# REGRAGUIahmed/DGViT-Depth-Goal-Guided-Vision-Transformer-

Measured on AMD Instinct MI355X. Metric: depth frames/sec through DGViT fwd+bwd, batch 512x84x84, higher is better.
Workload: dtype f32

## Files before the change

### dgvit-depth-goal-guided-vision-transformer-_amd/_lib.py

```python
import ctypes
import os
from ctypes import POINTER, Structure, c_char_p, c_float, c_int, c_longlong, c_ulonglong, c_void_p

_HERE = os.path.dirname(os.path.abspath(__file__))
LIB_PATH = os.path.join(_HERE, "libdgvit_hip.so")
DIAG_LIB_PATH = os.path.join(_HERE, "libdgvit_hip_diag.so")


class DgvitError(RuntimeError):
    pass


class dgvit_config(Structure):
    _fields_ = [("image_h", c_int), ("image_w", c_int), ("patch_h", c_int), ("patch_w", c_int), ("dim", c_int),
                ("depth", c_int), ("heads", c_int), ("dim_head", c_int), ("mlp_dim", c_int), ("pool_mean", c_int), ("flags", c_int)]


FLAG_DENSE_LAST_BLOCK = 1
FLAG_WGRAD_OVERLAP = 2
FLAG_LONG_SEQUENCE = 4
MAPS_GOAL = 0
MAPS_ALL = 1


# ... 124 lines not shown
    "dgvit_got_bf16_backward_scratch_bytes": (_LL, [_CFG, _I]),
    "dgvit_got_backward_bf16": (_I, [_CFG, _TABLE, _P, _TABLE, _P, _P, _P, _P, _LL, _P, _LL, _I, _F, _ULL, _P, _P]),
    "dgvit_got_backward_bf16_ev": (_I, [_CFG, _TABLE, _P, _TABLE, _P, _P, _P, _P, _LL, _P, _LL, _I, _F, _ULL, _P, _P, POINTER(dgvit_grad_events)]),
    "dgvit_got_backward_bf16_v2": (_I, [_CFG, _TABLE, _P, _TABLE, _P, _P, _P, _P, _P, _LL, _P, _LL, _I, _F, _ULL, _P, _P]),
    "dgvit_got_backward_bf16_v2_ev": (_I, [_CFG, _TABLE, _P, _TABLE, _P, _P, _P, _P, _P, _LL, _P, _LL, _I, _F, _ULL, _P, _P,
                                           POINTER(dgvit_grad_events)]),
    "dgvit_wgrad_bf16_scratch_floats": (_LL, [_I, _I, _I]),
    "dgvit_wgrad_bf16": (_I, [_P, _P, _P, _P, _P, _LL, _I, _I, _I, _P]),
    "dgvit_cast_f32_bf16": (_I, [_P, _P, _LL, _P]),
    "dgvit_gemm_bf16": (_I, [_I, _P, _I, _P, _I, _P, _I, _I, _I, _I, _P, _P, _I, _P, _I, _P, _I, _P]),
    "dgvit_layernorm_forward_bf16": (_I, [_P, _P, _P, _P, _P, _P, _I, _I, _P]),
    "dgvit_attention_forward_bf16": (_I, [_P, _P, _P, _I, _I, _I, _I, _P]),
    "dgvit_got_forward_maps": (_I, [_CFG, _TABLE, _P, _P, _P, _P, _I, _P, _LL, _I, _F, _F, _ULL, _P, _P]),
    "dgvit_got_forward_maps_bf16": (_I, [_CFG, _TABLE, _P, _P, _P, _P, _P, _I, _P, _LL, _I, _F, _ULL, _P, _P]),
    "dgvit_attention_probs": (_I, [_P, _P, _P, _I, _I, _I, _I, _I, _P]),
    "dgvit_attention_probs_bf16": (_I, [_P, _P, _P, _I, _I, _I, _I, _I, _P]),
    "dgvit_attention_backward_bf16": (_I, [_P, _P, _P, _P, _P, _P, _I, _I, _I, _I, _P]),
    "dgvit_attention_forward_bf16_tiled": (_I, [_P, _P, _P, _I, _I, _I, _I, _I, _P]),
    "dgvit_attention_backward_bf16_tiled": (_I, [_P, _P, _P, _P, _P, _P, _I, _I, _I, _I, _P]),
    "dgvit_got_forward_bf16_v2": (_I, [_CFG, _TABLE, _P, _P, _P, _P, _P, _LL, _I, _I, _F, _F, _ULL, _P, _P]),
    "dgvit_got_forward_maps_bf16_v2": (_I, [_CFG, _TABLE, _P, _P, _P, _P, _P, _I, _P, _LL, _I, _F, _F, _ULL, _P, _P]),
    "dgvit_got_backward_bf16_v3": (_I, [_CFG, _TABLE, _P, _TABLE, _P, _P, _P, _P, _P, _LL, _P, _LL, _I, _F, _F, _ULL, _P, _P]),
    "dgvit_got_backward_bf16_v3_ev": (_I, [_CFG, _TABLE, _P, _TABLE, _P, _P, _P, _P, _P, _LL, _P, _LL, _I, _F, _F, _ULL, _P, _P,
                                           POINTER(dgvit_grad_events)]),
    "dgvit_attention_forward_bf16_tiled_drop": (_I, [_P, _P, _P, _I, _I, _I, _I, _I, _F, _ULL, _P, _I, _P]),
    "dgvit_attention_backward_bf16_tiled_drop": (_I, [_P, _P, _P, _P, _P, _P, _I, _I, _I, _I, _F, _ULL, _P, _I, _P]),
    "dgvit_drop_rows_bf16": (_I, [_P, _LL, _P, _LL, _LL, _I, _I, _F, _ULL, _P, _I, _I, _P]),
    "dgvit_profile_start": (_I, [_I]),
    "dgvit_profile_stop": (_I, [POINTER(ctypes.c_double), POINTER(ctypes.c_double), POINTER(c_longlong)]),
    "dgvit_profile_sampling": (_I, [_I]),
    "dgvit_profile_totals": (_I, [POINTER(ctypes.c_double), POINTER(c_longlong)]),
}
DIAG_SIGNATURES = {
    "dgvit_set_gemm_tile": (None, [_I]),
    "dgvit_set_grouped_reduce": (None, [_I]),
    "dgvit_set_gemm_split": (None, [_I]),
    "dgvit_set_gemm_lds_pad": (None, [_I]),
    "dgvit_set_ln_fusion": (None, [_I]),
    "dgvit_set_conv_gather": (None, [_I]),
    "dgvit_set_gemm_diagnostics": (None, [_I]),
    "dgvit_set_gemm_persistent": (None, [_I, _I]),
    "dgvit_gemm_persistent_launches": (ctypes.c_longlong, []),
    "dgvit_set_gemm_stamps": (None, [_P, _I]),
    "dgvit_set_small_batch_path": (None, [_I, _I]),
    "dgvit_set_block_path": (None, [_I, _I]),
    "dgvit_set_block_stamps": (None, [_P]),
    "dgvit_set_block_stamp_layer": (None, [_I]),
    "dgvit_set_gelu_grad_store": (None, [_I]),
    "dgvit_set_block_fuse": (None, [_I]),
    "dgvit_set_gemm_bf16_tile": (None, [_I]),
    "dgvit_set_gemm_bf16_group_m": (None, [_I]),
    "dgvit_set_gemm_bf16_l2_budget_kb": (None, [_I]),
    "dgvit_set_attention_bwd_single_pass": (None, [_I]),
    "dgvit_set_attention_single_query": (None, [_I]),
    "dgvit_set_last_block_fold": (None, [_I]),
    "dgvit_set_attention_bf16_long": (None, [_I]),
    "dgvit_set_attention_bf16_tiled_waves": (None, [_I]),
    "dgvit_set_gemm_wgrad_slice_major": (None, [_I]),
    "dgvit_attention_forward_queries": (_I, [_P, _P, _P, _I, _I, _I, _I, _I, _P]),
    "dgvit_attention_backward_queries": (_I, [_P, _P, _P, _P, _P, _I, _I, _I, _I, _I, _P]),
    "dgvit_attention_forward_bf16_queries": (_I, [_P, _P, _P, _I, _I, _I, _I, _I, _P]),
    "dgvit_set_gemm_bf16_mfma16": (None, [_I]),
    "dgvit_set_gemm_bf16_stamps": (None, [_P]),
    "dgvit_diag_layernorm_forward": (_I, [_P, _P, _P, _P, _P, _P, _I, _I, _I, _P]),
    "dgvit_diag_layernorm_backward": (_I, [_P, _P, _P, _P, _P, _P, _P, _P, _P, _P, _LL, _I, _I, _I, _I, _P]),
    "dgvit_diag_layernorm_forward_bf16": (_I, [_P, _P, _P, _P, _P, _P, _P, _P, _P, _I, _I, _I, _P]),
    "dgvit_diag_layernorm_backward_bf16": (_I, [_P, _P, _P, _P, _P, _P, _P, _P, _P, _P, _P, _LL, _I, _I, _I, _P]),
    "dgvit_diag_residual_add_bf16": (_I, [_P, _P, _P, _I, _I, _I, _P]),
    "dgvit_diag_transpose_cast_f32_bf16": (_I, [_P, _P, _I, _I, _P]),
    "dgvit_diag_colsum_scratch_floats": (_LL, [_I, _I]),
    "dgvit_diag_colsum": (_I, [_P, _LL, _P, _P, _LL, _I, _I, _I, _P]),
}
PROFILE_KINDS = 4

_lib = None
_product = None
_diag = None


def _open(path, signatures):
    if not os.path.exists(path):
        raise DgvitError(f"{path} not found: build it with `python {os.path.join(_HERE, 'build.py')}` "
                         "(hipcc --offload-arch=gfx950). There is no fallback path.")
    lib = ctypes.CDLL(path)
    for name, (res, args) in signatures.items():
        try:
            fn = getattr(lib, name)
        except AttributeError as e:
            raise DgvitError(f"{path} does not export {name}; rebuild it") from e
        fn.restype, fn.argtypes = res, args
    if lib.dgvit_abi_version() != ABI_VERSION:
        raise DgvitError(f"ABI mismatch: library {lib.dgvit_abi_version()} != binding {ABI_VERSION}")
    if lib.dgvit_config_size() != ctypes.sizeof(dgvit_config):
        raise DgvitError(f"dgvit_config is {ctypes.sizeof(dgvit_config)} bytes in the binding, {lib.dgvit_config_size()} in the library")
    return lib


def load():
    global _lib, _product
    if _lib is not None:
        return _lib
    if _product is None:
        _product = _open(LIB_PATH, SIGNATURES)
    _lib = _product
    return _lib

# ... 23 lines not shown
```

### dgvit-depth-goal-guided-vision-transformer-_amd/csrc/attention.hip

```cpp
#include "common.h"
#include "kernels.h"
#include "attention_tiles.h"

namespace {

template <int DH, int NW, int NKT_CT, bool DROP = false>
__global__ void __launch_bounds__(64 * NW, 2) attn_fwd_kernel(const float* __restrict__ qkv, float* __restrict__ out,
                                                              float* __restrict__ lse, int N, int H, float scale, int nq,
                                                              const LayerDrop drop) {
  constexpr int SK = DH + 4, DT = DH / 32, NTHR = 64 * NW;
  extern __shared__ __attribute__((aligned(16))) float smem[];
  const int nkt = NKT_CT ? NKT_CT : (N + 31) / 32, NP = nkt * 32;
  float* Ks = smem;
  float* Vs = smem + NP * SK;
  const int tid = threadIdx.x, lane = tid & 63, wave = tid >> 6;
  const int li = lane & 31, h = lane >> 5;
  const int b = blockIdx.x / H, hd = blockIdx.x % H;
  const int I = H * DH;
  const long long ld = 3ll * I;
  const float* base = qkv + (long long)b * N * ld + hd * DH;
  const float qscale = scale * DGVIT_LOG2E;

  const int nqt = (nq + 31) / 32;
  float4 qf[DH / 8];
// ... 346 lines not shown
  __syncthreads();
  for (int kt = wave; kt < nkt; kt += NW) {
    const int key = kt * 32 + li;
    const bool kv = key < N;
    if (kt != wave) {
      const int kc = kv ? key : 0;
      row_frags<DH>(kf, base + I + kc * ld, kv, h, 1.f);
      row_frags<DH>(vf, base + 2 * I + kc * ld, kv, h, 1.f);
    }
    f32x16 dk[DT], dv[DT];
    zero_tiles<DT>(dk);
    zero_tiles<DT>(dv);
#pragma unroll 1
    for (int qt = 0; qt < nqt; ++qt) {
      f32x16 s, dp;
#pragma unroll
      for (int r = 0; r < 16; ++r) {
        s[r] = 0.f;
        dp[r] = 0.f;
      }
      mfma_rows_x_frags<DH, SK>(s, X, qt * 32 + li, h, kf);
      mfma_rows_x_frags<DH, SK>(dp, Y, qt * 32 + li, h, vf);
#pragma unroll
      for (int r = 0; r < 16; ++r) {
        const int q = qt * 32 + acc_row(r, h);
        const float pv = (kv && q < nq) ? __builtin_amdgcn_exp2f(s[r] * qscale - lse_s[q]) : 0.f;
        float mk = 1.f;
        if constexpr (DROP) {
          if (kv && q < nq) {
            const uint4 rb = drop_bits((((long long)b * H + hd) * N + q) * ((N + 3) / 4) + key / 4, drop_seed(drop), drop.tag);
            const int w = key & 3;
            mk = drop_factor(w == 0 ? rb.x : w == 1 ? rb.y : w == 2 ? rb.z : rb.w, drop.keep, 1.0f / drop.keep);
          }
        }
        const float ds = DROP ? pv * (dp[r] * mk - del_s[q]) * scale : pv * (dp[r] - del_s[q]) * scale;
        const float pd = DROP ? pv * mk : pv;
        const float* dorow = Y + q * SK + li;
        const float* qrow = X + q * SK + li;
#pragma unroll
        for (int dt = 0; dt < DT; ++dt) {
          dv[dt] = __builtin_amdgcn_mfma_f32_32x32x2f32(dorow[dt * 32], pd, dv[dt], 0, 0, 0);
          dk[dt] = __builtin_amdgcn_mfma_f32_32x32x2f32(qrow[dt * 32], ds, dk[dt], 0, 0, 0);
        }
      }
    }
    if (kv) {
      store_T<DH>(dk, gbase + I + key * ld, h, 1.f);
      store_T<DH>(dv, gbase + 2 * I + key * ld, h, 1.f);
    }
  }
}

template <int DH>
__global__ void __launch_bounds__(256, 3) attn_bwd64_kernel(const float* __restrict__ qkv, const float* __restrict__ o_fwd,
                                                            const float* __restrict__ d_out, const float* __restrict__ lse,
                                                            float* __restrict__ dqkv, int N, int H, float scale) {
  constexpr int SK = DH + 4, DT = DH / 32, NP = 64, TQ = NP + 4;
  extern __shared__ __attribute__((aligned(16))) float smem[];
  float* X = smem;
  float* Y = X + NP * SK;
  float* T = Y + NP * SK;
  const int tid = threadIdx.x, lane = tid & 63, wave = tid >> 6;
  const int li = lane & 31, h = lane >> 5;
  const int b = blockIdx.x / H, hd = blockIdx.x % H;
  const int I = H * DH;
  const long long ld = 3ll * I;
  const float* base = qkv + (long long)b * N * ld + hd * DH;
  const float* obase = o_fwd + (long long)b * N * I + hd * DH;
  const float* dobase = d_out + (long long)b * N * I + hd * DH;
  float* gbase = dqkv + (long long)b * N * ld + hd * DH;
  const float qscale = scale * DGVIT_LOG2E;
  f32x16 dsT;
  const int qt1 = wave & 1, kt1 = wave >> 1, q1 = qt1 * 32 + li;
  {
    const int qt = qt1, kt = kt1, q = q1;
    const bool qv = q < N;
    const int qc = qv ? q : 0;
    float4 qf[DH / 8], dof[DH / 8];
    float delta, lq;
    {
      constexpr int C4 = DH / 4, PER = NP * C4 / 256;
      float4 kst[PER], vst[PER];
#pragma unroll
      for (int j = 0; j < PER; ++j) {
        const int f = tid + j * 256, row = f / C4, c = (f % C4) * 4;
        const int rr = row < N ? row : 0;
        kst[j] = *reinterpret_cast<const float4*>(base + I + rr * ld + c);
        vst[j] = *reinterpret_cast<const float4*>(base + 2 * I + rr * ld + c);
      }
      float4 of[DH / 8];
      row_frags<DH>(qf, base + qc * ld, qv, h, qscale);
      row_frags<DH>(dof, dobase + (long long)qc * I, qv, h, 1.f);
      row_frags<DH>(of, obase + (long long)qc * I, qv, h, 1.f);
      lq = qv ? lse[((long long)b * H + hd) * N + qc] : 0.f;
#pragma unroll
      for (int j = 0; j < PER; ++j) {
        const int f = tid + j * 256, row = f / C4, c = (f % C4) * 4;
        const float k = row < N ? 1.f : 0.f;
        *reinterpret_cast<float4*>(X + row * SK + c) = make_float4(kst[j].x * k, kst[j].y * k, kst[j].z * k, kst[j].w * k);
        *reinterpret_cast<float4*>(Y + row * SK + c) = make_float4(vst[j].x * k, vst[j].y * k, vst[j].z * k, vst[j].w * k);
      }
      float d = 0.f;
#pragma unroll
      for (int g = 0; g < DH / 8; ++g) d += (dof[g].x * of[g].x + dof[g].y * of[g].y) + (dof[g].z * of[g].z + dof[g].w * of[g].w);
      delta = d + __shfl_xor(d, 32, 64);
    }
    __syncthreads();
    f32x16 sT, dpT;
#pragma unroll
// ... 81 lines not shown
        for (int dt = 0; dt < DT; ++dt) dv[dt] = __builtin_amdgcn_mfma_f32_32x32x2f32(dov[e][dt], pe[e], dv[dt], 0, 0, 0);
    }
    __syncthreads();
#pragma unroll
    for (int r = 0; r < 16; ++r) T[(kt1 * 32 + acc_row(r, h)) * TQ + q1] = dsT[r];
    __syncthreads();
#pragma unroll
    for (int g = 0; g < 4; ++g) {
      if (qt * 32 + 8 * g >= N) continue;
      const float4 sf = *reinterpret_cast<const float4*>(T + key * TQ + qt * 32 + 8 * g + 4 * h);
      const float se[4] = {sf.x, sf.y, sf.z, sf.w};
      float qv4[4][DT];
#pragma unroll
      for (int e = 0; e < 4; ++e) {
        const float* qrow = X + (qt * 32 + 8 * g + 4 * h + e) * SK + li;
#pragma unroll
        for (int dt = 0; dt < DT; ++dt) qv4[e][dt] = qrow[dt * 32];
      }
#pragma unroll
      for (int e = 0; e < 4; ++e)
#pragma unroll
        for (int dt = 0; dt < DT; ++dt) dk[dt] = __builtin_amdgcn_mfma_f32_32x32x2f32(qv4[e][dt], se[e], dk[dt], 0, 0, 0);
    }
    __syncthreads();
    float* ek = T + key * TQ;
    float* ev = X + key * SK;
    if (qt == 1) {
#pragma unroll
      for (int dt = 0; dt < DT; ++dt)
#pragma unroll
        for (int c = 0; c < 4; ++c) {
          *reinterpret_cast<float4*>(ek + dt * 32 + 8 * c + 4 * h) = make_float4(dk[dt][4 * c], dk[dt][4 * c + 1], dk[dt][4 * c + 2], dk[dt][4 * c + 3]);
          *reinterpret_cast<float4*>(ev + dt * 32 + 8 * c + 4 * h) = make_float4(dv[dt][4 * c], dv[dt][4 * c + 1], dv[dt][4 * c + 2], dv[dt][4 * c + 3]);
        }
    }
    __syncthreads();
    if (qt == 0 && key < N) {
      const float unscale = 1.f / qscale;
#pragma unroll
      for (int dt = 0; dt < DT; ++dt)
#pragma unroll
        for (int c = 0; c < 4; ++c) {
          const float4 a = *reinterpret_cast<const float4*>(ek + dt * 32 + 8 * c + 4 * h);
          const float4 bq = *reinterpret_cast<const float4*>(ev + dt * 32 + 8 * c + 4 * h);
          *reinterpret_cast<float4*>(gbase + I + key * ld + dt * 32 + 8 * c + 4 * h) =
              make_float4((dk[dt][4 * c] + a.x) * unscale, (dk[dt][4 * c + 1] + a.y) * unscale, (dk[dt][4 * c + 2] + a.z) * unscale,
                          (dk[dt][4 * c + 3] + a.w) * unscale);
          *reinterpret_cast<float4*>(gbase + 2 * I + key * ld + dt * 32 + 8 * c + 4 * h) =
              make_float4(dv[dt][4 * c] + bq.x, dv[dt][4 * c + 1] + bq.y, dv[dt][4 * c + 2] + bq.z, dv[dt][4 * c + 3] + bq.w);
        }
    }
  }
}


template <int DH>
int launch_bwd64(const float* qkv, const float* o, const float* dout, const float* lse, float* dqkv, int B, int N, int H, float scale,
                 hipStream_t stream) {
  constexpr size_t lds = (size_t)(2 * 64 * (DH + 4) + 64 * 68) * sizeof(float);
  auto kern = attn_bwd64_kernel<DH>;
  TRY(allow_dynamic_lds<attn_bwd64_kernel<DH>>((int)lds, "attention_bwd"));
  {
    ProfileScope t(PROF_ATTN_BWD, 8.0 * B * H * (double)N * N * DH, stream);
    hipLaunchKernelGGL(kern, dim3(B * H), dim3(256), lds, stream, qkv, o, dout, lse, dqkv, N, H, scale);
  }
  DGVIT_CHECK_LAUNCH("attention_bwd64");
  return DGVIT_OK;
}

template <int W>
__device__ __forceinline__ float lanes_sum(float v) {
#pragma unroll
  for (int o = W >> 1; o > 0; o >>= 1) v += __shfl_xor(v, o, 64);
  return v;
}
template <int W>
__device__ __forceinline__ float groups_sum(float v) {
#pragma unroll
  for (int o = W; o < 64; o <<= 1) v += __shfl_xor(v, o, 64);
  return v;
}
__device__ __forceinline__ float dot4(const float4 a, const float4 b) { return (a.x * b.x + a.y * b.y) + (a.z * b.z + a.w * b.w); }

template <int DH>
__global__ void __launch_bounds__(256) attn_q1_fwd_kernel(const float* __restrict__ qkv, float* __restrict__ out, float* __restrict__ lse,
                                                          int N, int H, float scale, int items) {
  constexpr int C4 = DH / 4, G = 64 / C4, NI = 64 / G;
  const int lane = threadIdx.x & 63, item = blockIdx.x * 4 + (threadIdx.x >> 6);
  if (item >= items) return;
  const int b = item / H, hd = item - b * H, I = H * DH;
  const long long ld = 3ll * I;
  const int c = lane % C4, g = lane / C4;
  const float* base = qkv + (long long)b * N * ld + hd * DH + 4 * c;
  float4 kf[NI], vf[NI];
#pragma unroll
  for (int i = 0; i < NI; ++i) {
    const int key = i * G + g, rr = key < N ? key : 0;
    kf[i] = *reinterpret_cast<const float4*>(base + I + rr * ld);
    vf[i] = *reinterpret_cast<const float4*>(base + 2 * I + rr * ld);
  }
  float4 q = *reinterpret_cast<const float4*>(base);
  const float qscale = scale * DGVIT_LOG2E;
  q = make_float4(q.x * qscale, q.y * qscale, q.z * qscale, q.w * qscale);
  float sc[NI], m = -INFINITY;
#pragma unroll
  for (int i = 0; i < NI; ++i) {
    const float d = lanes_sum<C4>(dot4(q, kf[i]));
    sc[i] = i * G + g < N ? d : -INFINITY;
    m = fmaxf(m, sc[i]);
  }
#pragma unroll
  for (int o = C4; o < 64; o <<= 1) m = fmaxf(m, __shfl_xor(m, o, 64));
  float l = 0.f;
  float4 o4 = make_float4(0.f, 0.f, 0.f, 0.f);
#pragma unroll
  for (int i = 0; i < NI; ++i) {
    const float pv = __builtin_amdgcn_exp2f(sc[i] - m);
// ... 92 lines not shown
}

template <int DH, int NW, int NKT_CT, bool DROP>
int launch_bwd(const float* qkv, const float* o, const float* dout, const float* lse, float* dqkv, int B, int N, int H,
               float scale, int nq, const LayerDrop& drop, hipStream_t stream) {
  const int NP = (N + 31) / 32 * 32;
  const size_t lds = ((size_t)2 * NP * (DH + 4) + 2 * NP) * sizeof(float);
  auto kern = attn_bwd_kernel<DH, NW, NKT_CT, DROP>;
  TRY((allow_dynamic_lds<attn_bwd_kernel<DH, NW, NKT_CT, DROP>>((2 * MAX_TOKENS * (DH + 4) + 2 * MAX_TOKENS) * (int)sizeof(float), "attention_bwd")));
  {
    ProfileScope t(PROF_ATTN_BWD, 8.0 * B * H * (double)nq * N * DH, stream);
    hipLaunchKernelGGL(kern, dim3(B * H), dim3(64 * NW), lds, stream, qkv, o, dout, lse, dqkv, N, H, scale, nq, drop);
  }
  DGVIT_CHECK_LAUNCH("attention_bwd");
  return DGVIT_OK;
}

}

#define ATTN_DISPATCH(FN, DROP, ...)                                      \
  {                                                                       \
    const int nt = (N + 31) / 32;                                         \
    if (dh == 64 && nt == 1) return FN<64, 1, 1, DROP>(__VA_ARGS__);      \
    if (dh == 64 && nt == 2) return FN<64, 2, 2, DROP>(__VA_ARGS__);      \
    if (dh == 64) return FN<64, 4, 0, DROP>(__VA_ARGS__);                 \
    if (dh == 32 && nt == 1) return FN<32, 1, 1, DROP>(__VA_ARGS__);      \
    if (dh == 32 && nt == 2) return FN<32, 2, 2, DROP>(__VA_ARGS__);      \
    if (dh == 32) return FN<32, 4, 0, DROP>(__VA_ARGS__);                 \
  }

int attention_fwd(const float* qkv, float* out, float* lse, int B, int N, int H, int dh, int nq, hipStream_t stream, const LayerDrop* drop) {
  DGVIT_CHECK_ARG(qkv && out && B > 0 && N > 0 && H > 0, "attention_fwd: bad arguments");
  DGVIT_CHECK_ARG((long long)B * H < (1ll << 31), "attention_fwd: B*H too large");
  DGVIT_CHECK_ARG(nq >= 1 && nq <= N, "attention_fwd: bad query count");
  DGVIT_CHECK_ARG(N <= MAX_TOKENS && (dh == 64 || dh == 32), "attention_fwd: unsupported dim_head=%d / tokens=%d (dim_head 64 or 32, N <= 288)", dh, N);
  const float scale = 1.0f / sqrtf((float)dh);
  const LayerDrop none = {1.f, 0u, 0ull, nullptr};
  if (drop && drop->keep < 1.f) {
    DGVIT_CHECK_ARG(drop->keep > 0.f, "attention_fwd: dropout keep must be in (0, 1]");
    ATTN_DISPATCH(launch_fwd, true, qkv, out, lse, B, N, H, scale, nq, *drop, stream)
  }
  if (g_attn_q1 && nq == 1 && N <= 64) {
    if (dh == 64) return launch_q1_fwd<64>(qkv, out, lse, B, N, H, scale, stream);
    return launch_q1_fwd<32>(qkv, out, lse, B, N, H, scale, stream);
  }
  if (nq == N && N > 32 && N <= 64 && (long long)B * H >= 2048) {
    if (dh == 64) return launch_fwd_pipe<64>(qkv, out, lse, B, N, H, scale, stream);
    return launch_fwd_pipe<32>(qkv, out, lse, B, N, H, scale, stream);
  }
  ATTN_DISPATCH(launch_fwd, false, qkv, out, lse, B, N, H, scale, nq, none, stream)
  return dgvit_set_error(DGVIT_ERR_ARG, "attention_fwd: no kernel for dim_head=%d", dh);
}


int attention_bwd(const float* qkv, const float* o, const float* dout, const float* lse, float* dqkv, int B, int N, int H,
                  int dh, int nq, hipStream_t stream, const LayerDrop* drop) {
  DGVIT_CHECK_ARG(qkv && o && dout && lse && dqkv && B > 0 && N > 0 && H > 0, "attention_bwd: bad arguments");
  DGVIT_CHECK_ARG((long long)B * H < (1ll << 31), "attention_bwd: B*H too large");
  DGVIT_CHECK_ARG(nq >= 1 && nq <= N, "attention_bwd: bad query count");
  DGVIT_CHECK_ARG(N <= MAX_TOKENS && (dh == 64 || dh == 32), "attention_bwd: unsupported dim_head=%d / tokens=%d", dh, N);
  const float scale = 1.0f / sqrtf((float)dh);
  const LayerDrop none = {1.f, 0u, 0ull, nullptr};
  if (drop && drop->keep < 1.f) {
    DGVIT_CHECK_ARG(drop->keep > 0.f, "attention_bwd: dropout keep must be in (0, 1]");
    ATTN_DISPATCH(launch_bwd, true, qkv, o, dout, lse, dqkv, B, N, H, scale, nq, *drop, stream)
  }
  if (g_attn_q1 && nq == 1 && N <= 64) {
    if (dh == 64) return launch_q1_bwd<64>(qkv, o, dout, lse, dqkv, B, N, H, scale, stream);
    return launch_q1_bwd<32>(qkv, o, dout, lse, dqkv, B, N, H, scale, stream);
  }
  if (g_attn_bwd64 && nq == N && N > 32 && N <= 64) {
    if (dh == 64) return launch_bwd64<64>(qkv, o, dout, lse, dqkv, B, N, H, scale, stream);
    return launch_bwd64<32>(qkv, o, dout, lse, dqkv, B, N, H, scale, stream);
  }
  ATTN_DISPATCH(launch_bwd, false, qkv, o, dout, lse, dqkv, B, N, H, scale, nq, none, stream)
  return dgvit_set_error(DGVIT_ERR_ARG, "attention_bwd: no kernel for dim_head=%d", dh);
}
```

### dgvit-depth-goal-guided-vision-transformer-_amd/csrc/diag_api.hip

```cpp
#define DGVIT_KNOB_DEFINE
#include "../../include/dgvit_hip_diag.h"
#include "schedule.h"
#include "bf16.h"

#ifndef DGVIT_DIAG
#error "diag_api.hip belongs to the diagnostic library only (-DDGVIT_DIAG)"
#endif

long long g_gemm_persist_launches = 0;

extern "C" void dgvit_set_gemm_tile(int tile) { g_gemm_tile_hint = tile; }
extern "C" void dgvit_set_grouped_reduce(int on) { g_group_reduce = on ? 1 : 0; }
extern "C" void dgvit_set_conv_gather(int on) { g_conv_gather = on ? 1 : 0; }
extern "C" void dgvit_set_ln_fusion(int on) { g_ln_fusion = on ? 1 : 0; }
extern "C" void dgvit_set_gemm_split(int on) { g_gemm_split = on ? 1 : 0; }
extern "C" void dgvit_set_gemm_stamps(long long* stamps, int workgroups) {
  g_gemm_stamps = stamps;
  g_gemm_stamp_capacity = stamps ? workgroups : 0;
}
extern "C" long long dgvit_gemm_persistent_launches(void) { return g_gemm_persist_launches; }
extern "C" void dgvit_set_gemm_persistent(int mode, int workgroups) {
  g_gemm_persist = mode < 0 ? 0 : (mode > 2 ? 2 : mode);
  g_gemm_persist_grid = workgroups > 0 ? workgroups : 0;
}
extern "C" void dgvit_set_gemm_diagnostics(int on) { g_gemm_diag = on & 0x3FFFFF; }
extern "C" void dgvit_set_gemm_lds_pad(int bytes) { g_gemm_lds_pad = bytes > 0 ? bytes : 0; }
extern "C" void dgvit_set_small_batch_path(int on, int max_rows) {
  g_small_path = on ? 1 : 0;
  if (max_rows > 0) g_small_path_max_rows = max_rows;
}
extern "C" void dgvit_set_block_path(int on, int max_rows) {
  g_block_path = on < 0 ? 0 : (on > 2 ? 2 : on);
  g_block_path_max_rows = max_rows > 0 ? max_rows : g_block_path_max_rows_default;
}
extern "C" void dgvit_set_block_stamps(long long* stamps) { g_block_stamps = stamps; }
extern "C" void dgvit_set_block_stamp_layer(int layer) { g_block_stamp_layer = layer; }
extern "C" void dgvit_set_gelu_grad_store(int on) { g_gelu_grad_store = on ? 1 : 0; }
extern "C" void dgvit_set_block_fuse(int bits) { g_block_fuse = bits & 3; }
extern "C" void dgvit_set_gemm_bf16_tile(int tile) { g_gemm_bf16_tile_hint = tile; }
extern "C" void dgvit_set_gemm_bf16_mfma16(int on) { g_gemm_bf16_m16 = on ? 1 : 0; }
extern "C" void dgvit_set_attention_bwd_single_pass(int on) { g_attn_bwd64 = on ? 1 : 0; }
extern "C" void dgvit_set_attention_single_query(int on) { g_attn_q1 = on ? 1 : 0; }
extern "C" void dgvit_set_last_block_fold(int on) { g_last_block_fold = on ? 1 : 0; }
extern "C" void dgvit_set_attention_bf16_tiled_waves(int waves) { g_attn_bf16_tiled_waves = waves == 8 ? 8 : waves == 4 ? 4 : g_attn_bf16_tiled_waves_default; }
extern "C" void dgvit_set_attention_bf16_long(int bits) { g_attn_bf16_long = bits < 0 ? g_attn_bf16_long_default : (bits & 3); }
extern "C" void dgvit_set_gemm_wgrad_slice_major(int on) { g_gemm_zfold = on ? 1 : 0; }
extern "C" int dgvit_attention_forward_queries(const float* qkv, float* out, float* lse, int B, int N, int H, int dh, int nq, void* stream) {
  return attention_fwd(qkv, out, lse, B, N, H, dh, nq, (hipStream_t)stream);
}
extern "C" int dgvit_attention_backward_queries(const float* qkv, const float* out, const float* dout, const float* lse, float* dqkv,
                                                int B, int N, int H, int dh, int nq, void* stream) {
  return attention_bwd(qkv, out, dout, lse, dqkv, B, N, H, dh, nq, (hipStream_t)stream);
}
extern "C" int dgvit_attention_forward_bf16_queries(const unsigned short* qkv, unsigned short* out, float* lse, int B, int N, int H, int dh,
                                                    int nq, void* stream) {
  return attention_fwd_bf16((const bf16_t*)qkv, (bf16_t*)out, lse, B, N, H, dh, nq, (hipStream_t)stream);
}
extern "C" void dgvit_set_gemm_bf16_group_m(int rows) { g_gemm_bf16_group_m = rows > 0 ? rows : g_gemm_bf16_group_m_default; }
extern "C" void dgvit_set_gemm_bf16_stamps(long long* stamps) { g_gemm_bf16_stamps = stamps; }
extern "C" void dgvit_set_gemm_bf16_l2_budget_kb(int kb) { g_gemm_bf16_l2_budget_kb = kb > 0 ? kb : 0; }

extern "C" int dgvit_diag_layernorm_forward(const float* x, const float* gamma, const float* beta, float* y, float* mean, float* rstd,
                                            int rows, int D, int row_step, void* stream) {
  return layernorm_fwd(x, gamma, beta, y, mean, rstd, rows, D, 1e-5f, row_step, (hipStream_t)stream);
}
extern "C" int dgvit_diag_layernorm_backward(const float* dy, const float* x, const float* mean, const float* rstd, const float* gamma,
                                             const float* dres, float* dx, float* dgamma, float* dbeta, float* scratch,
                                             long long scratch_floats, int rows, int D, int row_step, int grouped, void* stream) {
  if (rows <= 0 || D <= 0 || scratch_floats < (long long)layernorm_bwd_blocks(rows) * 2 * D)
    return dgvit_set_error(DGVIT_ERR_WORKSPACE, "diag_layernorm_backward: scratch too small");
  DGVIT_CHECK_ARG(row_step >= 1, "diag_layernorm_backward: bad row step");
  hipStream_t st = (hipStream_t)stream;
  if (!grouped) return layernorm_bwd(dy, x, mean, rstd, gamma, dres, dx, dgamma, dbeta, scratch, rows, D, row_step, st);
  ReduceGroup grp;
  reduce_group_init(grp);
  TRY(layernorm_bwd(dy, x, mean, rstd, gamma, dres, dx, dgamma, dbeta, scratch, rows, D, row_step, st, &grp));
  return reduce_group_flush(grp, st);
}
extern "C" int dgvit_diag_layernorm_forward_bf16(const float* x, const unsigned short* delta, const unsigned short* delta2, float* xout,
                                                 const float* gamma, const float* beta, unsigned short* y, float* mean, float* rstd,
                                                 int rows, int D, int row_step, void* stream) {
  hipStream_t st = (hipStream_t)stream;
  DGVIT_CHECK_ARG(row_step >= 1 && (mean == nullptr) == (rstd == nullptr), "diag_layernorm_forward_bf16: bad row step, or one of mean / rstd without the other");
  DGVIT_CHECK_ARG(delta || (!delta2 && !xout), "diag_layernorm_forward_bf16: delta2 / xout without delta");
  if (!delta) return layernorm_fwd_bf16(x, gamma, beta, y, mean, rstd, rows, D, 1e-5f, row_step, st);
  if (!delta2 && xout && mean) return add_layernorm_fwd_bf16(x, delta, xout, gamma, beta, y, mean, rstd, rows, D, 1e-5f, row_step, st);
  DGVIT_CHECK_ARG(row_step == 1 && !mean, "diag_layernorm_forward_bf16: the joint form has contiguous rows and no statistics");
  return add2_layernorm_fwd_bf16(x, delta, delta2, xout, gamma, beta, y, rows, D, 1e-5f, st);
}
extern "C" int dgvit_diag_layernorm_backward_bf16(const unsigned short* dy, const float* x, const float* mean, const float* rstd,
                                                  const float* gamma, const float* dres, float* dx, unsigned short* dxb, float* dgamma,
                                                  float* dbeta, float* scratch, long long scratch_floats, int rows, int D, int row_step,
                                                  void* stream) {
  if (rows <= 0 || D <= 0 || scratch_floats < (long long)layernorm_bwd_blocks(rows) * 2 * D)
// ... 24 lines not shown
```

### dgvit-depth-goal-guided-vision-transformer-_amd/csrc/kernels.h

```cpp
#pragma once
#include "common.h"

int layernorm_fwd(const float*, const float*, const float*, float*, float*, float*, int, int, float, int, hipStream_t);
int layernorm_bwd_blocks(int T);
int layernorm_bwd(const float*, const float*, const float*, const float*, const float*, const float*, float*, float*, float*,
                  float*, int, int, int, hipStream_t, ReduceGroup* grp = nullptr);
int rmsnorm_fwd(const float*, long long, const float*, float*, int, int, hipStream_t);
int rmsnorm_bwd_blocks(int B);
int rmsnorm_bwd(const float*, const float*, long long, const float*, float*, long long, float*, float*, int, int, hipStream_t);
int colsum_blocks(int T);
int colsum(const float*, long long, float*, float*, int, int, int, hipStream_t);
int attention_fwd(const float*, float*, float*, int, int, int, int, int, hipStream_t, const LayerDrop* drop = nullptr);
int attention_bwd(const float*, const float*, const float*, const float*, float*, int, int, int, int, int, hipStream_t,
                  const LayerDrop* drop = nullptr);
int attention_fwd_tiled(const float*, float*, float*, int, int, int, int, int, hipStream_t, const LayerDrop* drop = nullptr);
long long attention_bwd_tiled_scratch(int B, int N, int H);
int attention_bwd_tiled(const float*, const float*, const float*, const float*, float*, float*, long long, int, int, int, int, int,
                        hipStream_t, const LayerDrop* drop = nullptr);
int attention_probs(const float* qkv, const float* lse, float* probs, long long frame_stride, int B, int N, int H, int dh, int rows,
                    hipStream_t st);
constexpr long long GOAL_POOL_LDS_MAX = 159 * 1024;
constexpr long long GOAL_POOL_LDS_BUDGET = 80 * 1024;
long long goal_pool_lds_bytes(int N, int D, int H);
bool goal_attention_supports(int N, int D, int H, int dh);
int goal_attention_fwd(const float* xn, const float* wqkv, const float* q, long long ldq, float* o, long long ldo, float* u, float* r,
                       long long fs_ur, float* p, int B, int N, int H, int dh, int D, hipStream_t st);
int goal_attention_bwd_data(const float* xn, const float* wqkv, const float* dout, long long lddo, const float* u, long long fs_ur,
                            const float* p, float* du, float* dr, long long fs_d, float* dq, long long lddq, float* dxn, int B, int N, int H,
                            int dh, int D, hipStream_t st);
int goal_attention_wgrad(const float* q, long long ldq, const float* dout, long long lddo, const float* du, long long fs_d, const float* r,
                         long long fs_ur, float* dwkv, int B, int H, int dh, int D, hipStream_t st);
int patchify(const float*, float*, int, int, int, int, int, hipStream_t);
int add_rows(const float*, long long, const float*, long long, float*, long long, long long, int, hipStream_t);
int goal_row(const float*, const float*, float*, int, int, int, hipStream_t);
int dropout_inplace(float*, long long, unsigned long long, const unsigned long long*, float, hipStream_t);
int drop_rows(const float* src, long long lds, float* dst, long long ldd, const float* res, long long ldr, long long rows, int width, int rs,
              const LayerDrop& drop, hipStream_t stream);
int relu_bwd(const float*, const float*, float*, long long, hipStream_t);
int adam_step(float*, const float*, float*, float*, long long, float, float, float, float, float, long long, const long long*,
              hipStream_t);
int soft_update(float*, const float*, long long, float, hipStream_t);
int grad_sqnorm_partials(const float* g, long long n, double* partials, int accumulate, hipStream_t);
int grad_clip_coef(const double* partials, float max_norm, float* out, hipStream_t);
int adam_step_scaled(float*, const float*, float*, float*, long long, float, float, float, float, float, long long, const long long*,
                     const float* grad_scale_dev, hipStream_t);
int scale_by_device_scalar(float* x, long long n, const float* scale_dev, hipStream_t);
int adam_step_groups(float* p, const float* g, float* m, float* v, long long n, const long long* seg_end4, const unsigned char* seg_group,
                     int nseg, const float* group_hyper, int ngroups, float* lr_out, float beta1, float beta2, float eps, int decoupled,
                     long long step, long long sched_step, const long long* step_dev, int sched_kind, long long warmup_steps,
                     long long total_steps, float final_ratio, const float* grad_scale_dev, hipStream_t);
int sac_critic_loss(const float* q1, const float* q2, const float* reward, const float* done, const float* weights, const float* discount,
                    const float* next_q1, const float* next_q2, const float* next_log_pi, const float* log_alpha, float alpha, float gamma,
                    float* target, float* td, float* loss, float* grads, int B, int A, hipStream_t);
int sac_actor_loss(const float* log_pi, const float* q1_pi, const float* q2_pi, const float* log_alpha, float alpha, int with_temperature,
                   float target_entropy, float* losses, float* grads, float* dlog_alpha, int B, int A, hipStream_t);
int sac_scale_grads(const float* src, float* dst, long long n, const float* scale_dev, hipStream_t);
int im2col(const float*, float*, int, int, int, int, int, int, int, hipStream_t);
int col2im_relu(const float*, const float*, float*, int, int, int, int, int, int, hipStream_t);
int col2im_frame(const float*, float*, int, int, int, int, int, int, hipStream_t);
int weight_pack(const float*, float*, int, int, int, int, hipStream_t);
int avgpool(const float*, float*, int, int, int, hipStream_t);
int avgpool_bwd_relu(const float*, const float*, float*, int, int, int, hipStream_t);
int gather_rows(const float*, const long long*, float*, long long, long long, long long, hipStream_t);
int gather_shift_frames(const float* src, const long long* idx, float* out, int* shifts_out, long long nsel, int H, int W,
                        long long row_floats, long long nrows, int pad, int stream_id, unsigned long long seed,
                        const unsigned long long* seed_dev, hipStream_t stream);
int quantize_rows_u8(const float* src, long long src_ld, unsigned char* ring, long long n, long long cols, long long row_bytes,
// ... 64 lines not shown
```

### dgvit-depth-goal-guided-vision-transformer-_amd/csrc/knobs.h

```cpp
#pragma once

#ifdef DGVIT_DIAG
#ifdef DGVIT_KNOB_DEFINE
#define DGVIT_KNOB(type, name, def) type name = def; constexpr type name##_default = def;
#else
#define DGVIT_KNOB(type, name, def) extern type name;
#endif
#define DGVIT_DIAG_ONLY(...) __VA_ARGS__
#define KNOB_IF(k) if (k)
#else
#define DGVIT_KNOB(type, name, def) static constexpr type name = def;
#define DGVIT_DIAG_ONLY(...)
#define KNOB_IF(k) if constexpr ((k) != 0)
#endif

DGVIT_KNOB(int, g_gemm_tile_hint, 0)
DGVIT_KNOB(int, g_gemm_split, 1)
DGVIT_KNOB(int, g_gemm_lds_pad, 0)
DGVIT_KNOB(int, g_gemm_persist, 0)
DGVIT_KNOB(int, g_gemm_persist_grid, 0)
DGVIT_KNOB(int, g_gemm_diag, 0)
DGVIT_KNOB(long long*, g_gemm_stamps, nullptr)
DGVIT_KNOB(int, g_gemm_stamp_capacity, 0)
DGVIT_KNOB(int, g_group_reduce, 1)
DGVIT_KNOB(int, g_ln_fusion, 1)
DGVIT_KNOB(int, g_conv_gather, 1)
DGVIT_KNOB(int, g_gelu_grad_store, 1)
DGVIT_KNOB(int, g_block_path, 1)
DGVIT_KNOB(int, g_block_fuse, 2)
DGVIT_KNOB(int, g_block_path_max_rows, 4160)
DGVIT_KNOB(long long*, g_block_stamps, nullptr)
DGVIT_KNOB(int, g_block_stamp_layer, -1)
DGVIT_KNOB(int, g_block_stamp_now, 1)
DGVIT_KNOB(int, g_small_path, 0)
DGVIT_KNOB(int, g_small_path_max_rows, 4160)
DGVIT_KNOB(int, g_gemm_bf16_tile_hint, 0)
DGVIT_KNOB(int, g_gemm_bf16_m16, 1)
DGVIT_KNOB(int, g_gemm_bf16_group_m, 8)
DGVIT_KNOB(int, g_gemm_bf16_l2_budget_kb, 2048)
DGVIT_KNOB(long long*, g_gemm_bf16_stamps, nullptr)
DGVIT_KNOB(int, g_attn_bwd64, 1)
DGVIT_KNOB(int, g_gemm_zfold, 1)
DGVIT_KNOB(int, g_attn_q1, 1)
DGVIT_KNOB(int, g_attn_bf16_long, 3)
DGVIT_KNOB(int, g_attn_bf16_tiled_waves, 8)
DGVIT_KNOB(int, g_last_block_fold, 1)
#ifdef DGVIT_DIAG
extern long long g_gemm_persist_launches;
#endif
```

### include/dgvit_hip_diag.h

```cpp
#ifndef DGVIT_HIP_DIAG_H
#define DGVIT_HIP_DIAG_H
#include "dgvit_hip.h"

#ifdef __cplusplus
extern "C" {
#endif
#pragma GCC visibility push(default)

void dgvit_set_gemm_tile(int tile);
void dgvit_set_grouped_reduce(int on);
void dgvit_set_gemm_split(int on);
void dgvit_set_ln_fusion(int on);
void dgvit_set_conv_gather(int on);
void dgvit_set_gemm_lds_pad(int bytes);
void dgvit_set_gemm_diagnostics(int bits);
void dgvit_set_gemm_persistent(int mode, int workgroups);
long long dgvit_gemm_persistent_launches(void);
void dgvit_set_gemm_stamps(long long* stamps, int workgroups);
void dgvit_set_small_batch_path(int on, int max_rows);
void dgvit_set_block_path(int on, int max_rows);
void dgvit_set_block_stamps(long long* stamps);
void dgvit_set_block_stamp_layer(int layer);
void dgvit_set_gelu_grad_store(int on);
void dgvit_set_block_fuse(int bits);
void dgvit_set_gemm_bf16_tile(int tile);
void dgvit_set_gemm_bf16_group_m(int rows);
void dgvit_set_gemm_bf16_l2_budget_kb(int kb);
void dgvit_set_attention_bwd_single_pass(int on);
void dgvit_set_attention_single_query(int on);
void dgvit_set_last_block_fold(int on);
void dgvit_set_attention_bf16_long(int bits);
void dgvit_set_attention_bf16_tiled_waves(int waves);
void dgvit_set_gemm_wgrad_slice_major(int on);
int dgvit_attention_forward_queries(const float* qkv, float* out, float* lse, int B, int N, int H, int dh, int nq, void* stream);
int dgvit_attention_backward_queries(const float* qkv, const float* out, const float* dout, const float* lse, float* dqkv, int B, int N, int H,
                                     int dh, int nq, void* stream);
int dgvit_attention_forward_bf16_queries(const unsigned short* qkv, unsigned short* out, float* lse, int B, int N, int H, int dh, int nq,
                                         void* stream);
void dgvit_set_gemm_bf16_mfma16(int on);
void dgvit_set_gemm_bf16_stamps(long long* stamps);

int dgvit_diag_layernorm_forward(const float* x, const float* gamma, const float* beta, float* y, float* mean, float* rstd, int rows, int D,
                                 int row_step, void* stream);
int dgvit_diag_layernorm_backward(const float* dy, const float* x, const float* mean, const float* rstd, const float* gamma, const float* dres,
                                  float* dx, float* dgamma, float* dbeta, float* scratch, long long scratch_floats, int rows, int D,
                                  int row_step, int grouped, void* stream);
int dgvit_diag_layernorm_forward_bf16(const float* x, const unsigned short* delta, const unsigned short* delta2, float* xout,
                                      const float* gamma, const float* beta, unsigned short* y, float* mean, float* rstd, int rows, int D,
                                      int row_step, void* stream);
int dgvit_diag_layernorm_backward_bf16(const unsigned short* dy, const float* x, const float* mean, const float* rstd, const float* gamma,
                                       const float* dres, float* dx, unsigned short* dxb, float* dgamma, float* dbeta, float* scratch,
                                       long long scratch_floats, int rows, int D, int row_step, void* stream);
int dgvit_diag_residual_add_bf16(const float* x, const unsigned short* delta, float* xout, int rows, int D, int row_step, void* stream);
int dgvit_diag_transpose_cast_f32_bf16(const float* src, unsigned short* dst, int rows, int cols, void* stream);
long long dgvit_diag_colsum_scratch_floats(int rows, int cols);
int dgvit_diag_colsum(const float* a, long long lda, float* out, float* scratch, long long scratch_floats, int rows, int cols, int rgrp,
                      void* stream);

#pragma GCC visibility pop
#ifdef __cplusplus
}
#endif
#endif
```

Before: 41460.

## Shrink attention backward LDS footprint by aliasing K/V/dO images to raise occupancy

```diff
diff --git a/dgvit-depth-goal-guided-vision-transformer-_amd/_lib.py b/dgvit-depth-goal-guided-vision-transformer-_amd/_lib.py
--- a/dgvit-depth-goal-guided-vision-transformer-_amd/_lib.py
+++ b/dgvit-depth-goal-guided-vision-transformer-_amd/_lib.py
@@ -200,6 +200,8 @@
     "dgvit_set_gemm_bf16_group_m": (None, [_I]),
     "dgvit_set_gemm_bf16_l2_budget_kb": (None, [_I]),
     "dgvit_set_attention_bwd_single_pass": (None, [_I]),
+    "dgvit_set_attn_bwd64_compact": (None, [_I]),
+    "dgvit_attn_bwd64_lds_bytes": (_LL, [_I, _I]),
     "dgvit_set_attention_single_query": (None, [_I]),
     "dgvit_set_last_block_fold": (None, [_I]),
     "dgvit_set_attention_bf16_long": (None, [_I]),
diff --git a/dgvit-depth-goal-guided-vision-transformer-_amd/csrc/attention.hip b/dgvit-depth-goal-guided-vision-transformer-_amd/csrc/attention.hip
--- a/dgvit-depth-goal-guided-vision-transformer-_amd/csrc/attention.hip
+++ b/dgvit-depth-goal-guided-vision-transformer-_amd/csrc/attention.hip
@@ -422,9 +422,262 @@
 }
 
 template <int DH>
-__global__ void __launch_bounds__(256, 3) attn_bwd64_kernel(const float* __restrict__ qkv, const float* __restrict__ o_fwd,
-                                                            const float* __restrict__ d_out, const float* __restrict__ lse,
-                                                            float* __restrict__ dqkv, int N, int H, float scale) {
+constexpr size_t attn_bwd64_lds(bool compact) {
+  return compact ? (size_t)(64 * (DH + 4) + 64 * 68 + 4 * 64) * sizeof(float) : (size_t)(2 * 64 * (DH + 4) + 64 * 68) * sizeof(float);
+}
+
+template <int DH, bool DELTA_O>
+__device__ __forceinline__ void attn_bwd64_body(const float* __restrict__ qkv, const float* __restrict__ o_fwd,
+                                                const float* __restrict__ d_out, const float* __restrict__ lse,
+                                                float* __restrict__ dqkv, int N, int H, float scale) {
+  constexpr int SK = DH + 4, DT = DH / 32, NP = 64, TQ = NP + 4;
+  static_assert(SK <= TQ, "the V image lives in the [64][68] region");
+  extern __shared__ __attribute__((aligned(16))) float smem[];
+  float* R1 = smem;
+  float* R2 = R1 + NP * SK;
+  float* DX = R2 + NP * TQ;
+  const int tid = threadIdx.x, lane = tid & 63, wave = tid >> 6;
+  const int li = lane & 31, h = lane >> 5;
+  const int b = blockIdx.x / H, hd = blockIdx.x % H;
+  const int I = H * DH;
+  const long long ld = 3ll * I;
+  const float* base = qkv + (long long)b * N * ld + hd * DH;
+  const float* dobase = d_out + (long long)b * N * I + hd * DH;
+  float* gbase = dqkv + (long long)b * N * ld + hd * DH;
+  const float qscale = scale * DGVIT_LOG2E;
+  f32x16 dsT;
+  float4 keep[DH / 8];
+  const int qt1 = wave & 1, kt1 = wave >> 1, q1 = qt1 * 32 + li;
+  {
+    const int qt = qt1, kt = kt1, q = q1;
+    const bool qv = q < N;
+    const int qc = qv ? q : 0;
+    f32x16 sT, dpT;
+    float delta = 0.f, lq;
+    {
+      float4 first[DH / 8];
+      const float* qrow = base + qc * ld;
+      const float* dorow = dobase + (long long)qc * I;
+      const float* img1 = kt ? R2 : R1;
+      const float* img2 = kt ? R1 : R2;
+      {
+        constexpr int C4 = DH / 4, PER = NP * C4 / 256;
+        float4 kst[PER], vst[PER];
+#pragma unroll
+        for (int j = 0; j < PER; ++j) {
+          const int f = tid + j * 256, row = f / C4, c = (f % C4) * 4;
+          const int rr = row < N ? row : 0;
+          kst[j] = *reinterpret_cast<const float4*>(base + I + rr * ld + c);
+          vst[j] = *reinterpret_cast<const float4*>(base + 2 * I + rr * ld + c);
+        }
+        row_frags<DH>(first, kt ? dorow : qrow, true, h, 1.f);
+        row_frags<DH>(keep, kt ? qrow : dorow, true, h, 1.f);
+        lq = qv ? lse[((long long)b * H + hd) * N + qc] : 0.f;
+#pragma unroll
+        for (int j = 0; j < PER; ++j) {
+          const int f = tid + j * 256, row = f / C4, c = (f % C4) * 4;
+          const float k = row < N ? 1.f : 0.f;
+          *reinterpret_cast<float4*>(R1 + row * SK + c) = make_float4(kst[j].x * k, kst[j].y * k, kst[j].z * k, kst[j].w * k);
+          *reinterpret_cast<float4*>(R2 + row * SK + c) = make_float4(vst[j].x * k, vst[j].y * k, vst[j].z * k, vst[j].w * k);
+        }
+      }
+      if constexpr (DELTA_O) {
+        const float* orow = o_fwd + (long long)b * N * I + hd * DH + (long long)qc * I;
+        float4 of[DH / 8];
+        row_frags<DH>(of, orow, qv, h, 1.f);
+        float d = 0.f;
+#pragma unroll
+        for (int g = 0; g < DH / 8; ++g) {
+          const float4 dg = make_float4(kt ? first[g].x : keep[g].x, kt ? first[g].y : keep[g].y, kt ? first[g].z : keep[g].z,
+                                        kt ? first[g].w : keep[g].w);
+          d += (dg.x * of[g].x + dg.y * of[g].y) + (dg.z * of[g].z + dg.w * of[g].w);
+        }
+        delta = d + __shfl_xor(d, 32, 64);
+      }
+      __syncthreads();
+      f32x16 a1, a2;
+#pragma unroll
+      for (int r = 0; r < 16; ++r) {
+        a1[r] = 0.f;
+        a2[r] = 0.f;
+      }
+      mfma_rows_x_frags<DH, SK>(a1, img1, kt * 32 + li, h, first);
+      mfma_rows_x_frags<DH, SK>(a2, img2, kt * 32 + li, h, keep);
+#pragma unroll
+      for (int r = 0; r < 16; ++r) {
+        sT[r] = kt ? a2[r] : a1[r];
+        dpT[r] = kt ? a1[r] : a2[r];
+      }
+    }
+    float part = 0.f, psum = 0.f;
+#pragma unroll
+    for (int r = 0; r < 16; ++r) {
+      const int key = kt * 32 + acc_row(r, h);
+      const float pv = (qv && key < N) ? __builtin_amdgcn_exp2f(sT[r] * qscale - lq) : 0.f;
+      sT[r] = pv;
+      part += pv * dpT[r];
+      psum += pv;
+    }
+    if constexpr (!DELTA_O) {
+      part += __shfl_xor(part, 32, 64);
+      psum += __shfl_xor(psum, 32, 64);
+      if (h == 0) {
+        DX[kt * NP + q] = part;
+        DX[(2 + kt) * NP + q] = psum;
+      }
+    }
+    __syncthreads();
+    if constexpr (!DELTA_O) {
+      const float rinv = qv ? 1.f / (DX[2 * NP + q] + DX[3 * NP + q]) : 0.f;
+      delta = (DX[q] + DX[NP + q]) * rinv;
+#pragma unroll
+      for (int r = 0; r < 16; ++r) sT[r] *= rinv;
+    }
+#pragma unroll
+    for (int r = 0; r < 16; ++r) {
+      const int key = kt * 32 + acc_row(r, h);
+      R2[key * TQ + q] = sT[r];
+      dsT[r] = sT[r] * (dpT[r] - delta) * scale;
+    }
+    f32x16 dq[DT];
+    zero_tiles<DT>(dq);
+#pragma unroll
+    for (int g4 = 0; g4 < 4; ++g4) {
+      if (kt * 32 + 8 * g4 >= N) continue;
+      float kv[4][DT];
+#pragma unroll
+      for (int r4 = 0; r4 < 4; ++r4) {
+        const float* krow = R1 + (kt * 32 + acc_row(4 * g4 + r4, h)) * SK + li;
+#pragma unroll
+        for (int dt = 0; dt < DT; ++dt) kv[r4][dt] = krow[dt * 32];
+      }
+#pragma unroll
+      for (int r4 = 0; r4 < 4; ++r4)
+#pragma unroll
+        for (int dt = 0; dt < DT; ++dt) dq[dt] = __builtin_amdgcn_mfma_f32_32x32x2f32(kv[r4][dt], dsT[4 * g4 + r4], dq[dt], 0, 0, 0);
+    }
+    __syncthreads();
+    float* ex = R1 + q * SK;
+    if (kt == 1) {
+#pragma unroll
+      for (int dt = 0; dt < DT; ++dt)
+#pragma unroll
+        for (int c = 0; c < 4; ++c)
+          *reinterpret_cast<float4*>(ex + dt * 32 + 8 * c + 4 * h) = make_float4(dq[dt][4 * c], dq[dt][4 * c + 1], dq[dt][4 * c + 2], dq[dt][4 * c + 3]);
+    }
+    __syncthreads();
+    if (kt == 0) {
+      if (qv) {
+#pragma unroll
+        for (int dt = 0; dt < DT; ++dt)
+#pragma unroll
+          for (int c = 0; c < 4; ++c) {
+            const float4 o = *reinterpret_cast<const float4*>(ex + dt * 32 + 8 * c + 4 * h);
+            *reinterpret_cast<float4*>(gbase + q * ld + dt * 32 + 8 * c + 4 * h) =
+                make_float4(dq[dt][4 * c] + o.x, dq[dt][4 * c + 1] + o.y, dq[dt][4 * c + 2] + o.z, dq[dt][4 * c + 3] + o.w);
+          }
+      }
+#pragma unroll
+      for (int g = 0; g < DH / 8; ++g) *reinterpret_cast<float4*>(ex + 8 * g + 4 * h) = keep[g];
+    }
+    __syncthreads();
+  }
+  {
+    const int kt = wave & 1, qt = wave >> 1;
+    const int key = kt * 32 + li;
+    f32x16 dk[DT], dv[DT];
+    zero_tiles<DT>(dv);
+#pragma unroll
+    for (int g = 0; g < 4; ++g) {
+      if (qt * 32 + 8 * g >= N) continue;
+      const float4 pf = *reinterpret_cast<const float4*>(R2 + key * TQ + qt * 32 + 8 * g + 4 * h);
+      const float pe[4] = {pf.x, pf.y, pf.z, pf.w};
+      float dov[4][DT];
+#pragma unroll
+      for (int e = 0; e < 4; ++e) {
+        const float* dorow = R1 + (qt * 32 + 8 * g + 4 * h + e) * SK + li;
+#pragma unroll
+        for (int dt = 0; dt < DT; ++dt) dov[e][dt] = dorow[dt * 32];
+      }
+#pragma unroll
+      for (int e = 0; e < 4; ++e)
+#pragma unroll
+        for (int dt = 0; dt < DT; ++dt) dv[dt] = __builtin_amdgcn_mfma_f32_32x32x2f32(dov[e][dt], pe[e], dv[dt], 0, 0, 0);
+    }
+    __syncthreads();
+#pragma unroll
+    for (int r = 0; r < 16; ++r) R2[(kt1 * 32 + acc_row(r, h)) * TQ + q1] = dsT[r];
+    if (kt1 == 1) {
+#pragma unroll
+      for (int g = 0; g < DH / 8; ++g) *reinterpret_cast<float4*>(R1 + q1 * SK + 8 * g + 4 * h) = keep[g];
+    }
+    __syncthreads();
+    zero_tiles<DT>(dk);
+#pragma unroll
+    for (int g = 0; g < 4; ++g) {
+      if (qt * 32 + 8 * g >= N) continue;
+      const float4 sf = *reinterpret_cast<const float4*>(R2 + key * TQ + qt * 32 + 8 * g + 4 * h);
+      const float se[4] = {sf.x, sf.y, sf.z, sf.w};
+      float qv4[4][DT];
+#pragma unroll
+      for (int e = 0; e < 4; ++e) {
+        const float* qrow = R1 + (qt * 32 + 8 * g + 4 * h + e) * SK + li;
+#pragma unroll
+        for (int dt = 0; dt < DT; ++dt) qv4[e][dt] = qrow[dt * 32];
+      }
+#pragma unroll
+      for (int e = 0; e < 4; ++e)
+#pragma unroll
+        for (int dt = 0; dt < DT; ++dt) dk[dt] = __builtin_amdgcn_mfma_f32_32x32x2f32(qv4[e][dt], se[e], dk[dt], 0, 0, 0);
+    }
+    __syncthreads();
+    float* ek = R2 + key * TQ;
+    float* ev = R1 + key * SK;
+    if (qt == 1) {
+#pragma unroll
+      for (int dt = 0; dt < DT; ++dt)
+#pragma unroll
+        for (int c = 0; c < 4; ++c) {
+          *reinterpret_cast<float4*>(ek + dt * 32 + 8 * c + 4 * h) = make_float4(dk[dt][4 * c], dk[dt][4 * c + 1], dk[dt][4 * c + 2], dk[dt][4 * c + 3]);
+          *reinterpret_cast<float4*>(ev + dt * 32 + 8 * c + 4 * h) = make_float4(dv[dt][4 * c], dv[dt][4 * c + 1], dv[dt][4 * c + 2], dv[dt][4 * c + 3]);
+        }
+    }
+    __syncthreads();
+    if (qt == 0 && key < N) {
+#pragma unroll
+      for (int dt = 0; dt < DT; ++dt)
+#pragma unroll
+        for (int c = 0; c < 4; ++c) {
+          const float4 a = *reinterpret_cast<const float4*>(ek + dt * 32 + 8 * c + 4 * h);
+          const float4 bq = *reinterpret_cast<const float4*>(ev + dt * 32 + 8 * c + 4 * h);
+          *reinterpret_cast<float4*>(gbase + I + key * ld + dt * 32 + 8 * c + 4 * h) =
+              make_float4(dk[dt][4 * c] + a.x, dk[dt][4 * c + 1] + a.y, dk[dt][4 * c + 2] + a.z, dk[dt][4 * c + 3] + a.w);
+          *reinterpret_cast<float4*>(gbase + 2 * I + key * ld + dt * 32 + 8 * c + 4 * h) =
+              make_float4(dv[dt][4 * c] + bq.x, dv[dt][4 * c + 1] + bq.y, dv[dt][4 * c + 2] + bq.z, dv[dt][4 * c + 3] + bq.w);
+        }
+    }
+  }
+}
+
+template <int DH>
+__global__ void __launch_bounds__(256, DH == 64 ? 4 : 5) attn_bwd64_kernel(const float* __restrict__ qkv, const float* __restrict__ o_fwd,
+                                                                           const float* __restrict__ d_out, const float* __restrict__ lse,
+                                                                           float* __restrict__ dqkv, int N, int H, float scale) {
+  attn_bwd64_body<DH, false>(qkv, o_fwd, d_out, lse, dqkv, N, H, scale);
+}
+
+#ifdef DGVIT_DIAG
+template <int DH>
+__global__ void __launch_bounds__(256, DH == 64 ? 4 : 5) attn_bwd64_delta_o_kernel(const float* __restrict__ qkv, const float* __restrict__ o_fwd,
+                                                                                   const float* __restrict__ d_out, const float* __restrict__ lse,
+                                                                                   float* __restrict__ dqkv, int N, int H, float scale) {
+  attn_bwd64_body<DH, true>(qkv, o_fwd, d_out, lse, dqkv, N, H, scale);
+}
+
+template <int DH>
+__global__ void __launch_bounds__(256, 3) attn_bwd64_wide_kernel(const float* __restrict__ qkv, const float* __restrict__ o_fwd,
+                                                                 const float* __restrict__ d_out, const float* __restrict__ lse,
+                                                                 float* __restrict__ dqkv, int N, int H, float scale) {
   constexpr int SK = DH + 4, DT = DH / 32, NP = 64, TQ = NP + 4;
   extern __shared__ __attribute__((aligned(16))) float smem[];
   float* X = smem;
@@ -612,17 +865,30 @@
     }
   }
 }
+#endif
 
 
 template <int DH>
 int launch_bwd64(const float* qkv, const float* o, const float* dout, const float* lse, float* dqkv, int B, int N, int H, float scale,
                  hipStream_t stream) {
-  constexpr size_t lds = (size_t)(2 * 64 * (DH + 4) + 64 * 68) * sizeof(float);
+  constexpr size_t lds = attn_bwd64_lds<DH>(true);
   auto kern = attn_bwd64_kernel<DH>;
+  size_t bytes = lds;
+#ifdef DGVIT_DIAG
+  TRY((allow_dynamic_lds<attn_bwd64_kernel<DH>, attn_bwd64_delta_o_kernel<DH>, attn_bwd64_wide_kernel<DH>>((int)attn_bwd64_lds<DH>(false),
+                                                                                                          "attention_bwd")));
+  if (g_attn_bwd64_compact == 0) {
+    kern = attn_bwd64_wide_kernel<DH>;
+    bytes = attn_bwd64_lds<DH>(false);
+  } else if (g_attn_bwd64_compact == 2) {
+    kern = attn_bwd64_delta_o_kernel<DH>;
+  }
+#else
   TRY(allow_dynamic_lds<attn_bwd64_kernel<DH>>((int)lds, "attention_bwd"));
+#endif
   {
     ProfileScope t(PROF_ATTN_BWD, 8.0 * B * H * (double)N * N * DH, stream);
-    hipLaunchKernelGGL(kern, dim3(B * H), dim3(256), lds, stream, qkv, o, dout, lse, dqkv, N, H, scale);
+    hipLaunchKernelGGL(kern, dim3(B * H), dim3(256), bytes, stream, qkv, o, dout, lse, dqkv, N, H, scale);
   }
   DGVIT_CHECK_LAUNCH("attention_bwd64");
   return DGVIT_OK;
@@ -821,6 +1087,11 @@
   return dgvit_set_error(DGVIT_ERR_ARG, "attention_fwd: no kernel for dim_head=%d", dh);
 }
 
+long long attention_bwd64_lds_bytes(int dh, int arm) {
+  if (dh != 64 && dh != 32) return -1;
+  return (long long)(dh == 64 ? attn_bwd64_lds<64>(arm != 0) : attn_bwd64_lds<32>(arm != 0));
+}
+
 
 int attention_bwd(const float* qkv, const float* o, const float* dout, const float* lse, float* dqkv, int B, int N, int H,
                   int dh, int nq, hipStream_t stream, const LayerDrop* drop) {
diff --git a/dgvit-depth-goal-guided-vision-transformer-_amd/csrc/diag_api.hip b/dgvit-depth-goal-guided-vision-transformer-_amd/csrc/diag_api.hip
--- a/dgvit-depth-goal-guided-vision-transformer-_amd/csrc/diag_api.hip
+++ b/dgvit-depth-goal-guided-vision-transformer-_amd/csrc/diag_api.hip
@@ -40,6 +40,8 @@
 extern "C" void dgvit_set_gemm_bf16_tile(int tile) { g_gemm_bf16_tile_hint = tile; }
 extern "C" void dgvit_set_gemm_bf16_mfma16(int on) { g_gemm_bf16_m16 = on ? 1 : 0; }
 extern "C" void dgvit_set_attention_bwd_single_pass(int on) { g_attn_bwd64 = on ? 1 : 0; }
+extern "C" void dgvit_set_attn_bwd64_compact(int arm) { g_attn_bwd64_compact = arm == 0 || arm == 2 ? arm : g_attn_bwd64_compact_default; }
+extern "C" long long dgvit_attn_bwd64_lds_bytes(int dh, int arm) { return attention_bwd64_lds_bytes(dh, arm); }
 extern "C" void dgvit_set_attention_single_query(int on) { g_attn_q1 = on ? 1 : 0; }
 extern "C" void dgvit_set_last_block_fold(int on) { g_last_block_fold = on ? 1 : 0; }
 extern "C" void dgvit_set_attention_bf16_tiled_waves(int waves) { g_attn_bf16_tiled_waves = waves == 8 ? 8 : waves == 4 ? 4 : g_attn_bf16_tiled_waves_default; }
diff --git a/dgvit-depth-goal-guided-vision-transformer-_amd/csrc/kernels.h b/dgvit-depth-goal-guided-vision-transformer-_amd/csrc/kernels.h
--- a/dgvit-depth-goal-guided-vision-transformer-_amd/csrc/kernels.h
+++ b/dgvit-depth-goal-guided-vision-transformer-_amd/csrc/kernels.h
@@ -13,6 +13,7 @@
 int attention_fwd(const float*, float*, float*, int, int, int, int, int, hipStream_t, const LayerDrop* drop = nullptr);
 int attention_bwd(const float*, const float*, const float*, const float*, float*, int, int, int, int, int, hipStream_t,
                   const LayerDrop* drop = nullptr);
+long long attention_bwd64_lds_bytes(int dh, int arm);
 int attention_fwd_tiled(const float*, float*, float*, int, int, int, int, int, hipStream_t, const LayerDrop* drop = nullptr);
 long long attention_bwd_tiled_scratch(int B, int N, int H);
 int attention_bwd_tiled(const float*, const float*, const float*, const float*, float*, float*, long long, int, int, int, int, int,
diff --git a/dgvit-depth-goal-guided-vision-transformer-_amd/csrc/knobs.h b/dgvit-depth-goal-guided-vision-transformer-_amd/csrc/knobs.h
--- a/dgvit-depth-goal-guided-vision-transformer-_amd/csrc/knobs.h
+++ b/dgvit-depth-goal-guided-vision-transformer-_amd/csrc/knobs.h
@@ -40,6 +40,7 @@
 DGVIT_KNOB(int, g_gemm_bf16_l2_budget_kb, 2048)
 DGVIT_KNOB(long long*, g_gemm_bf16_stamps, nullptr)
 DGVIT_KNOB(int, g_attn_bwd64, 1)
+DGVIT_KNOB(int, g_attn_bwd64_compact, 1)
 DGVIT_KNOB(int, g_gemm_zfold, 1)
 DGVIT_KNOB(int, g_attn_q1, 1)
 DGVIT_KNOB(int, g_attn_bf16_long, 3)
diff --git a/include/dgvit_hip_diag.h b/include/dgvit_hip_diag.h
--- a/include/dgvit_hip_diag.h
+++ b/include/dgvit_hip_diag.h
@@ -27,6 +27,8 @@
 void dgvit_set_gemm_bf16_group_m(int rows);
 void dgvit_set_gemm_bf16_l2_budget_kb(int kb);
 void dgvit_set_attention_bwd_single_pass(int on);
+void dgvit_set_attn_bwd64_compact(int arm);
+long long dgvit_attn_bwd64_lds_bytes(int dh, int arm);
 void dgvit_set_attention_single_query(int on);
 void dgvit_set_last_block_fold(int on);
 void dgvit_set_attention_bf16_long(int bits);
```

Result: no change. 41580, median of 3 (+0.3%).
